# SegoleneMartin/transductive-CLIP

Measured on AMD Instinct MI355X. Metric: transductive tasks/sec (75-query EM-Dirichlet), higher is better.
Workload: dtype f32

## Files before the change

include/tclip.h:

```cpp
#ifndef TCLIP_H
#define TCLIP_H

#include <stddef.h>
#include <stdint.h>

#ifdef __cplusplus
extern "C" {
#endif

#define TCLIP_ABI_VERSION 5

enum {
    TCLIP_OK = 0,
    TCLIP_ERR_ARG = 1,
    TCLIP_ERR_WORKSPACE = 2,
    TCLIP_ERR_HIP = 3,
    TCLIP_ERR_INDEX = 4
};

typedef struct tclip_problem {
    int32_t n_batches;
    int32_t tasks_per_batch;
    int32_t n_query;
    int32_t n_class;
// ... 81 lines not shown
    float alpha_value;
    float loss_weights[3];
    int32_t entropies[3];
} tclip_tim_params;
size_t tclip_alpha_tim_workspace_bytes(const tclip_problem* p);
int tclip_alpha_tim_run(const tclip_problem* p, const tclip_tim_params* prm, const float* x_q, const float* x_s,
                        const int64_t* y_s, float* weights, float* logits_q, int32_t* preds, float* criterions,
                        void* workspace, size_t workspace_bytes, void* stream);

size_t tclip_laplacian_shot_workspace_bytes(const tclip_problem* p);
int tclip_laplacian_shot_run(const tclip_problem* p, const float* x_q, const float* x_s, const int64_t* y_s, int32_t knn,
                             double lmd, int32_t norm_type, float* unary, int32_t* neighbours, int32_t* preds_iter,
                             double* energies, void* workspace, size_t workspace_bytes, void* stream);

int tclip_argmax_rows(const float* x, int64_t n_rows, int32_t n_class, int32_t* labels, void* stream);

int tclip_probability_features(const float* visual, const float* text, int64_t n_rows, int32_t dim, int32_t n_class,
                               float temperature, float* out, void* stream);

#define TCLIP_VISUAL_SOFT_KMEANS 0
#define TCLIP_VISUAL_HARD_KMEANS 1
#define TCLIP_VISUAL_EM_GAUSSIAN 2
size_t tclip_visual_workspace_bytes(const tclip_problem* p, int32_t dim);
int tclip_kmeans_visual_run(const tclip_problem* p, int32_t dim, int32_t method, const float* x_q, const float* u0,
                            float temperature, float* u, float* v, float* w, int32_t* preds, float* criterions, void* workspace,
                            size_t workspace_bytes, void* stream);

int tclip_cluster_prototypes_visual(int32_t n_task, int32_t n_query, int32_t n_class, int32_t dim, const float* x_q,
                                    const int32_t* preds, int32_t* n_clusters, int32_t* cluster_ids, float* prototypes, void* stream);

int tclip_visual_init(const float* visual, const float* text, int64_t n_rows, int32_t dim, int32_t n_class,
                      float temperature, float* out, void* stream);

size_t tclip_paddle_visual_workspace_bytes(const tclip_problem* p, int32_t dim);
int tclip_paddle_visual_run(const tclip_problem* p, int32_t dim, const float* x_q, const float* x_s, const int64_t* y_s,
                            float lambd, float* u, float* v, float* w, int32_t* preds, void* workspace, size_t workspace_bytes,
                            void* stream);
size_t tclip_bdcspn_visual_workspace_bytes(const tclip_problem* p, int32_t dim);
int tclip_bdcspn_visual_run(const tclip_problem* p, int32_t dim, const float* x_q, const float* x_s, const int64_t* y_s, float temp,
                            int32_t norm_type, float* prototypes, float* u, int32_t* preds, void* workspace,
                            size_t workspace_bytes, void* stream);

int tclip_profile_enable(int on);
int tclip_profile_collect(double* mm_busy_ms, double* mm_launch_ms_sum, int64_t* mm_launches,
                          int64_t* element_updates);
int tclip_profile_last_kernels(double* busy_ms, double* launch_ms_sum, int64_t* launches, int64_t* element_updates);
int tclip_profile_last_split_sorts(int64_t* wave_iterations, int64_t* sorts);
int tclip_debug_set_split_keep_placement(int32_t on);

int tclip_debug_set_probe_chunks(int32_t chunks);

int tclip_debug_set_dead_head(int32_t iterations);

int tclip_debug_set_rowset_min_rows(int32_t rows);

int tclip_debug_set_mm_split(int32_t mode);

int tclip_debug_set_fixed_k_kernels(int32_t on);

int tclip_debug_set_kmeans_tile(int32_t mode);

int tclip_selftest_primitives(uint64_t* mismatches);

#ifdef __cplusplus
}
#endif
#endif
```

transductive-clip_amd/csrc/tclip_kernels.hip:

```cpp
#include <hip/hip_runtime.h>
#include <stdint.h>
#include <stdio.h>
#include <stdlib.h>
#include <string.h>

#include <algorithm>
#include <mutex>
#include <utility>
#include <vector>

#include "../../include/tclip.h"
#include "tclip_device.h"
#include "tclip_pk.h"
#include "tclip_selftest_inputs.h"

namespace tclip {

constexpr int kG64MinK = 897;

__global__ void k_log_features(const float* __restrict__ x, float* __restrict__ out, size_t n, int32_t* __restrict__ nonfinite) {
    bool bad = false;
    for (size_t i = (size_t)blockIdx.x * blockDim.x + threadIdx.x; i < n; i += (size_t)gridDim.x * blockDim.x) {
        const float v = log_f32(x[i] + kEpsF);
        out[i] = v;
// ... 278 lines not shown
        if (kCov) {
            y[row * K + d] = c / (s < kEpsF ? kEpsF : s);
        } else if (paddle == 2) {
            y[row * K + d] = s / c;
        } else if (sup && paddle) {
            y[row * K + d] = (s + sup[row * K + d]) / (c + cnt[row]);
        } else if (sup) {
            const float w = 1.0f / (cnt[row] + c);
            y[row * K + d] = w * (sup[row * K + d] + s);
        } else {
            y[row * K + d] = s / (c < kEpsF ? kEpsF : c);
        }
    }
}

__device__ __forceinline__ int lanes_below_mask(unsigned long long m, int lane) { return __popcll(m & ((1ull << lane) - 1ull)); }

__global__ void k_build_rows(const uint8_t* __restrict__ live, const int32_t* __restrict__ cache_len, int n_rows,
                             int n_checks, int32_t* __restrict__ dead_rows, int32_t* __restrict__ live_rows,
                             int32_t* __restrict__ n_dead, int32_t* __restrict__ n_live) {
    const int i = blockIdx.x * blockDim.x + threadIdx.x;
    const bool in = i < n_rows;
    const bool alive = in && live[i];
    const bool need = in && !alive && n_checks > 0 && cache_len[i] < n_checks;
    const unsigned long long ml = __ballot(alive), md = __ballot(need);
    const int lane64 = threadIdx.x & 63;
    int base_l = 0, base_d = 0;
    if (lane64 == 0) {
        if (ml) base_l = atomicAdd(n_live, __popcll(ml));
        if (md) base_d = atomicAdd(n_dead, __popcll(md));
    }
    base_l = __shfl(base_l, 0, 64);
    base_d = __shfl(base_d, 0, 64);
    if (alive) live_rows[base_l + lanes_below_mask(ml, lane64)] = i;
    if (need) dead_rows[base_d + lanes_below_mask(md, lane64)] = i;
}

struct MMArgs {
    float* alpha;
    float* beta_dead;
    const float* y;
    const uint8_t* live;
    int32_t* cache_len;
    double* cache;
    double* rowpart;
    const int32_t* rows;
    const int32_t* n_rows;
    const int32_t* stop;
    unsigned long long* work_counter;
    int32_t* next_rows;
    int32_t* next_count;
    int K, rows_per_batch, chunk, l0, l1, has_check, n_checks;
    int keep_placement;
};

constexpr int kYRegsMaxE = 16;
template <int E, int G>
__device__ __forceinline__ int elem_of(int e, int lane) {
    if constexpr (G == 64) return (lane >> 5) * (E * 32) + e * 32 + (lane & 31);
    else return e * G + lane;
}
template <int E, int G>
__host__ __device__ constexpr int full_registers(int K) {
    if constexpr (G == 64) return K > E * 32 ? (K - E * 32) / 32 : 0;
    else return K / G;
}

template <int E, int G = kGroup, int kRegsMaxE = kYRegsMaxE>
struct RowY {
    static constexpr bool kInRegs = E <= kRegsMaxE;
    float r[kInRegs ? E : 1];
    const float* g;
    int lane, K, n_full;
    __device__ __forceinline__ void load(const float* row_y, int lane_, int K_) {
        g = row_y; lane = lane_; K = K_; n_full = full_registers<E, G>(K_);
        if (kInRegs) {
#pragma unroll
            for (int e = 0; e < (kInRegs ? E : 1); e++) {
                const int d = elem_of<E, G>(e, lane);
                r[e] = d < K ? (g ? g[d] : -10.0f) : 0.0f;
            }
        }
    }
    __device__ __forceinline__ void fetch_all(float (&out)[E]) const {
        if (!g) {
#pragma unroll
            for (int e = 0; e < E; e++) out[e] = -10.0f;
            return;
        }
        if constexpr (G == 64) {
            const float* base = g;
            asm volatile("" : "+s"(base));
            const __amdgpu_buffer_rsrc_t rsrc = __builtin_amdgcn_make_buffer_rsrc((void*)base, 0, K * 4, 0x00020000);
            int voff = elem_of<E, G>(0, lane) * 4;
            asm volatile("" : "+v"(voff));
#pragma unroll
            for (int e = 0; e < E; e++) out[e] = __builtin_bit_cast(float, __builtin_amdgcn_raw_buffer_load_b32(rsrc, voff + e * 128, 0, 0));
        } else {
#pragma unroll
            for (int e = 0; e < E; e++) out[e] = get(e);
        }
    }
    __device__ __forceinline__ float get(int e) const {
        if (kInRegs) return r[kInRegs ? e : 0];
        if (!g) return -10.0f;
        const int d = elem_of<E, G>(e, lane);
// ... 158 lines not shown
    if constexpr (G == kGroup) return group_sum_torch<E, false, sure_registers<E, G, KC>()>(x, K, lane);
    else if constexpr (G == 64) return group_sum_torch_64<E, false, sure_registers<E, G, KC>()>(x, K, lane);
    else return group_sum_torch_g<E, G, false, sure_registers<E, G, KC>()>(x, K, lane);
}

template <int E, int G>
__device__ __forceinline__ void mm_iterate(float (&beta)[E], const RowY<E, G>& yv, int K, int lane,
                                           const LogTabEntry* tab, float* queue, bool measure, double& num,
                                           double& den) {
    const float s = row_sum_torch_all<E, G>(beta, K, lane);
    bool in_domain = fast_range_f32(s) && s <= 0x1p40f;
    uint32_t largest = 0u;
#pragma unroll
    for (int e = 0; e < E; e++) largest = max(largest, f32_bits(beta[e]));
    in_domain = in_domain & mm_fast_domain_of_max_bits(largest);
    if (__builtin_expect(!__all(in_domain), 0)) {
        const float psi_s = digamma_f32(s);
#pragma unroll
        for (int e = 0; e < E; e++) {
            const float nb = mm_update_generic(beta[e], yv.get(e), psi_s);
            const bool ok = elem_of<E, G>(e, lane) < K;
            if (measure && ok) {
                const double df = (double)nb - (double)beta[e];
                num += df * df;
                den += (double)beta[e] * (double)beta[e];
            }
            beta[e] = ok ? nb : 0.0f;
        }
        return;
    }
    const float psi_s = digamma_pos_f32(s, tab);
    int n_big = 0;
#pragma unroll
    for (int e = 0; e < E; e++) {
        const float x1 = beta[e] + 1.0f;
        const bool big = x1 >= 2.3f;
        const unsigned long long m = __ballot(big);
        if (big) queue[n_big + lanes_below(m)] = x1;
        n_big += __popcll(m);
    }
    __builtin_amdgcn_wave_barrier();
    const unsigned long long active = __ballot(true);
    const int rank = lanes_below(active), n_active = __popcll(active);
    for (int start = 0; start < n_big; start += n_active) {
        const int idx = start + rank;
        const float v = idx < n_big ? queue[idx] : 8.0f;
        const float r = lgamma_big_dense(v);
        if (idx < n_big) queue[idx] = r;
    }
    __builtin_amdgcn_wave_barrier();
    if (n_big == 0) mm_apply_updates_small<E, G>(beta, yv, K, lane, psi_s, tab, measure, num, den);
    else mm_apply_updates<E, G>(beta, yv, K, lane, psi_s, tab, queue, 0, measure, num, den);
    __builtin_amdgcn_wave_barrier();
}

constexpr int kProbeChunks = 2;
constexpr int kMaxCycle = 64;

constexpr int kMMWavesLarge = 3;
constexpr int kMMWavesSmall = 4;
template <int E, int G>
__global__ __launch_bounds__(256, (E > 16 ? kMMWavesLarge : kMMWavesSmall)) void k_mm_probe(MMArgs a) {
    __shared__ LogTabEntry tab[16];
    __shared__ double cyc[256 / G][kMaxCycle][2];
    __shared__ float lg_queue[4][64 * E];
    load_log_table(tab);
    float* queue = lg_queue[threadIdx.x >> 6];
    const int lane = threadIdx.x & (G - 1);
    const int group = threadIdx.x / G;
    const int groups_per_block = blockDim.x / G;
    const int n = *a.n_rows;
    const int K = a.K;
    for (int i = blockIdx.x * groups_per_block + group; i < n; i += gridDim.x * groups_per_block) {
        const int row = a.rows[i];
        if (a.stop[row / a.rows_per_batch]) continue;
        const int have = a.cache_len[row];
        if (have != a.chunk + 1) {
            if (a.next_rows && have < a.n_checks && lane == 0) a.next_rows[atomicAdd(a.next_count, 1)] = row;
            continue;
        }
        const float* ref = a.beta_dead + (size_t)row * K;
        float beta[E];
        RowY<E, G> yv;
        yv.load(nullptr, lane, K);
#pragma unroll
        for (int e = 0; e < E; e++) {
            const int d = elem_of<E, G>(e, lane);
            beta[e] = d < K ? ref[d] : 0.0f;
        }
        int period = 0;
        for (int j = 0; j < kMaxCycle && period == 0; j++) {
            double pn = 0.0, pd = 0.0;
            mm_iterate<E, G>(beta, yv, K, lane, tab, queue, true, pn, pd);
            pn = group_sum_f64_g<G>(pn);
            pd = group_sum_f64_g<G>(pd);
            if (lane == 0) { cyc[group][j][0] = pn; cyc[group][j][1] = pd; }
            bool same = true;
#pragma unroll
            for (int e = 0; e < E; e++) {
                const int d = elem_of<E, G>(e, lane);
                if (d < K) same = same && (beta[e] == ref[d]);
            }
            const unsigned long long bal = __ballot(same);
            constexpr unsigned long long kAll = G == 64 ? ~0ull : (1ull << (G & 63)) - 1ull;
            const unsigned long long mine = (bal >> ((threadIdx.x & 63) & ~(G - 1))) & kAll;
            if (mine == kAll) period = j + 1;
        }
        if (period && lane == 0) {
            for (int m = a.chunk + 1; m < a.n_checks; m++) {
                const int j = (50 * (m + 1) - (a.l1 + 1)) % period;
                double* c = a.cache + ((size_t)row * a.n_checks + m) * 2;
                c[0] = cyc[group][j][0];
                c[1] = cyc[group][j][1];
            }
            a.cache_len[row] = a.n_checks;
        }
        if (!period && a.next_rows && lane == 0) a.next_rows[atomicAdd(a.next_count, 1)] = row;
    }
}

constexpr int kDeadHead = 12;
static_assert(kDeadHead <= 18, "the last snapshot (32 iterations after the head) must lie at or before the first checkpoint (iteration 50)");
template <int E, int G>
__global__ __launch_bounds__(256, (E > 16 ? kMMWavesLarge : kMMWavesSmall)) void k_mm_probe_head(MMArgs a) {
    __shared__ LogTabEntry tab[16];
    __shared__ double cyc[256 / G][kMaxCycle][2];
    __shared__ float lg_queue[4][64 * E];
    load_log_table(tab);
    float* queue = lg_queue[threadIdx.x >> 6];
    const int lane = threadIdx.x & (G - 1);
    const int group = threadIdx.x / G;
    const int groups_per_block = blockDim.x / G;
    const int n = *a.n_rows;
    const int K = a.K;
    for (int i = blockIdx.x * groups_per_block + group; i < n; i += gridDim.x * groups_per_block) {
        const int row = a.rows[i];
        if (a.stop[row / a.rows_per_batch]) continue;
        if (a.cache_len[row] != 0) {
            if (lane == 0) a.next_rows[atomicAdd(a.next_count, 1)] = row;
            continue;
        }
        float* ref = a.beta_dead + (size_t)row * K;
        float* ref8 = const_cast<float*>(a.y) + (size_t)row * K;
        float beta[E];
        RowY<E, G> yv;
        yv.load(nullptr, lane, K);
#pragma unroll
        for (int e = 0; e < E; e++) {
            const int d = elem_of<E, G>(e, lane);
            beta[e] = d < K ? ref[d] : 0.0f;
        }
        int period = 0, js = 0, base = 0;
        bool have8 = false;
        constexpr unsigned long long kAll = G == 64 ? ~0ull : (1ull << (G & 63)) - 1ull;
        const int shift = (threadIdx.x & 63) & ~(G - 1);
        for (int j = 0; j < kMaxCycle && period == 0; j++) {
            double pn = 0.0, pd = 0.0;
            mm_iterate<E, G>(beta, yv, K, lane, tab, queue, true, pn, pd);
            pn = group_sum_f64_g<G>(pn);
            pd = group_sum_f64_g<G>(pd);
            if (lane == 0) { cyc[group][j][0] = pn; cyc[group][j][1] = pd; }
            bool same = true, same8 = have8;
#pragma unroll
            for (int e = 0; e < E; e++) {
                const int d = elem_of<E, G>(e, lane);
                if (d < K) same = same && (beta[e] == ref[d]);
            }
            if (have8) {
#pragma unroll
                for (int e = 0; e < E; e++) {
                    const int d = elem_of<E, G>(e, lane);
                    if (d < K) same8 = same8 && (beta[e] == ref8[d]);
                }
            }
            const bool hit = ((__ballot(same) >> shift) & kAll) == kAll, hit8 = ((__ballot(same8) >> shift) & kAll) == kAll;
            if (hit) {
                period = j + 1 - js;
                base = js;
            } else if (have8 && hit8) {
                period = j + 1 - 8;
                base = 8;
            } else if (j + 1 == 8 || j + 1 == 32) {
                float* dst = j + 1 == 8 ? ref8 : ref;
#pragma unroll
                for (int e = 0; e < E; e++) {
                    const int d = elem_of<E, G>(e, lane);
                    if (d < K) dst[d] = beta[e];
                }
                if (j + 1 == 8) have8 = true;
                else js = 32;
            }
        }
        if (period && lane == 0) {
            for (int m = 0; m < a.n_checks; m++) {
                const int t = 50 * (m + 1) - a.l0;
                const int j = base + (t - base) % period;
                double* c = a.cache + ((size_t)row * a.n_checks + m) * 2;
                c[0] = cyc[group][j][0];
                c[1] = cyc[group][j][1];
            }
            a.cache_len[row] = a.n_checks;
        }
        if (!period && lane == 0) a.next_rows[atomicAdd(a.next_count, 1)] = row;
    }
}

struct QueueCtl { int count[2][8]; int bad; float rowsum[2][64]; float psi[2][64]; };

template <int E, int G, int KC = 0>
__device__ __forceinline__ float row_sum_torch(const float (&x)[E], int K, int lane) {
    if constexpr (G == kGroup) return group_sum_torch<E, true, sure_registers<E, G, KC>()>(x, K, lane);
    else if constexpr (G == 64) return group_sum_torch_64<E, true, sure_registers<E, G, KC>()>(x, K, lane);
    else return group_sum_torch_g<E, G, true, sure_registers<E, G, KC>()>(x, K, lane);
}

template <int E, int W, int R, int G, int KC = 0>
__device__ __forceinline__ void mm_iterate_block(float (&beta)[R][E], const RowY<E, G> (&yv)[R], int K, int lane,
                                                 const bool (&active)[R], const LogTabEntry* tab, float* queue, QueueCtl* ctl,
                                                 int turn, bool measure, double (&num)[R], double (&den)[R]) {
    constexpr int kGroups = (64 / G) * W;
    const int wave = threadIdx.x >> 6, lane64 = threadIdx.x & 63;
    float s[R];
    bool in_domain = true;
    float* slice = queue + wave * (64 * E * R);
    int base[R + 1];
    base[0] = 0;
#pragma unroll
    for (int r = 0; r < R; r++) {
        s[r] = 16.0f;
        if (active[r]) {
            s[r] = row_sum_torch<E, G, KC>(beta[r], K, lane);
            in_domain = in_domain && (lane != 0 || (fast_range_f32(s[r]) && s[r] <= 0x1p40f));
            uint32_t largest = 0u;
#pragma unroll
            for (int e = 0; e < E; e++) largest = max(largest, f32_bits(beta[r][e]));
            in_domain = in_domain & mm_fast_domain_of_max_bits(largest);
        }
        if (lane == 0) ctl->rowsum[turn & 1][r * kGroups + (threadIdx.x / G)] = s[r];
        int idx = base[r];
#pragma unroll
        for (int e = 0; e < E; e++) {
            const float x1 = beta[r][e] + 1.0f;
            const bool big = active[r] && x1 >= 2.3f;
// ... 1510 lines not shown
        }
        if (x1 >= 2.3f) b2 += f32_bits(digamma_rec_acc_ge23(x1)) != f32_bits(acc);
        b2 += f32_bits(psip.x) != f32_bits(digamma_pos_f32(xp.x, tab)) || f32_bits(psip.y) != f32_bits(digamma_pos_f32(xp.y, tab));
    }
    for (uint32_t m = tid; m < (1u << 24); m += nth) {
        const float x = bits_f32(0x3f800000u + m);
        const f2 r = pk_sqrt_torch_inrange(f2{x, x * 0x1p-60f});
        b4 += f32_bits(r.x) != f32_bits(sqrt_torch_inrange_f32(x)) || f32_bits(r.y) != f32_bits(sqrt_torch_inrange_f32(x * 0x1p-60f));
        b4 += f32_bits(sqrt_torch_inrange_dev(x * 0x1p61f)) != f32_bits(sqrt_torch_inrange_f32(x * 0x1p61f));
    }
    for (int e = -100 + (int)tid; e <= 100; e += (int)nth) {
        const float x = bits_f32((uint32_t)(127 + e) << 23);
        b4 += f32_bits(sqrt_torch_inrange_dev(x)) != f32_bits(sqrt_torch_inrange_f32(x));
        b4 += f32_bits(pk_sqrt_torch_inrange(pk(x)).y) != f32_bits(sqrt_torch_inrange_f32(x));
    }
    atomicAdd(&out[0], b0); atomicAdd(&out[1], b1); atomicAdd(&out[2], b2);
    atomicAdd(&out[3], b3); atomicAdd(&out[4], b4); atomicAdd(&out[5], b5);
    for (int f = 0; f < kSelfTestFunctions; f++) {
        unsigned long long c = 0;
        for (uint32_t i = tid; i < kSelfTestCount; i += nth) c += selftest_term(f, i, tab);
        atomicAdd(&out[6 + f], c);
    }
}

thread_local char g_err[512] = "";

static int fail(int code, const char* fmt, const char* detail = "") {
    snprintf(g_err, sizeof g_err, fmt, detail);
    return code;
}

#define TCLIP_HIP(call)                                                                     \
    do {                                                                                    \
        hipError_t e_ = (call);                                                             \
        if (e_ != hipSuccess) return fail(TCLIP_ERR_HIP, #call ": %s", hipGetErrorString(e_)); \
    } while (0)

static size_t align_up(size_t x) { return (x + 255) & ~(size_t)255; }

struct Profile {
    bool on = false;
    std::vector<hipEvent_t> ev;
    std::vector<uint8_t> kind;
    size_t used = 0;
    unsigned long long* counter = nullptr;
    double last_busy[2] = {0, 0}, last_sum[2] = {0, 0};
    int64_t last_launches[2] = {0, 0}, last_updates[2] = {0, 0};
    int64_t last_split_iterations = 0, last_split_sorts = 0;
};
static thread_local bool g_last_mm_was_split = false;
thread_local Profile g_prof;
static int g_probe_chunks = kProbeChunks;
static int g_dead_head = kDeadHead;
static int g_rowset_min_rows = -1;
static int g_mm_split = -1;
static int g_split_keep_placement = 1;

static hipEvent_t prof_event() {
    if (g_prof.used == g_prof.ev.size()) {
        hipEvent_t e;
        if (hipEventCreate(&e) != hipSuccess) return nullptr;
        g_prof.ev.push_back(e);
    }
    return g_prof.ev[g_prof.used++];
}

constexpr int kDecideSlices = 64;
struct Layout {
    size_t logz, y, alpha_old, beta_dead, sup, cnt, cs, live, rowc, logit0, cache, cache_len, rowpart, mm_rows,
        mm_rows2, mm_rows3, dead_counts, cls, n_live, live_rows, counts, flags, stop, ratio, dpart, total;
    int n_checks;
};

static int n_chunks_of(int iter_mm) { return iter_mm <= 51 ? 1 : 1 + (iter_mm - 51 + 49) / 50; }
static int n_checks_of(int iter_mm) { return iter_mm <= 50 ? 0 : (iter_mm - 1) / 50; }

static Layout make_layout(const tclip_problem& p) {
    Layout L;
    const size_t T = (size_t)p.n_batches * p.tasks_per_batch, K = p.n_class, Q = p.n_query;
    const bool zs = p.n_support == 0;
    L.n_checks = n_checks_of(p.iter_mm);
    size_t o = 0;
    auto take = [&](size_t bytes) { size_t r = o; o += align_up(bytes); return r; };
    L.logz = take(T * Q * K * 4);
    L.y = take(T * K * K * 4);
    L.alpha_old = take(T * K * K * 4);
    L.beta_dead = take(zs ? T * K * K * 4 : 0);
    L.sup = take(zs ? 0 : T * K * K * 4);
    L.cnt = take(zs ? 0 : T * K * 4);
    L.cs = take(T * K * 4);
    L.live = take(T * K);
    L.rowc = take(T * K * 4);
    L.logit0 = take(T * Q * K * 4);
    L.cache = take(zs ? T * K * (size_t)L.n_checks * 16 : 0);
    L.cache_len = take(T * K * 4);
    L.rowpart = take(T * K * 16);
    L.mm_rows = take(T * K * 4);
    L.mm_rows2 = take(zs ? T * K * 4 : 0);
    L.mm_rows3 = take(zs ? T * K * 4 : 0);
    L.dead_counts = take(((size_t)n_chunks_of(p.iter_mm) + 3) * 4);
    L.cls = take(zs ? T * K * 2 : 0);
    L.n_live = take(zs ? T * 4 : 0);
    L.live_rows = take(T * K * 4);
    L.counts = take(256);
    L.flags = take(256);
    L.stop = take((size_t)p.n_batches * 4);
// ... 572 lines not shown
    int32_t* counts = (int32_t*)(ws + L.counts);
    int32_t* flags = (int32_t*)(ws + L.flags);
    int32_t* stop = (int32_t*)(ws + L.stop);
    float* ratio = (float*)(ws + L.ratio);
    double* dpart = (double*)(ws + L.dpart);
    const int n_chunks = n_chunks_of(p.iter_mm);
    const int n_checks = zs ? L.n_checks : 0;

    TCLIP_HIP(hipMemsetAsync(flags, 0, 256, st));
    if (q_src.idx) {
        const size_t rows = (size_t)T * Q;
        hipLaunchKernelGGL(k_gather_log_features, dim3((unsigned)(rows > 65536 ? 65536 : rows)), dim3(256), 0, st, q_src, Q, K, rows, u, logz, flags);
    } else {
        hipLaunchKernelGGL(k_log_features, dim3(ew_grid(TQK)), dim3(256), 0, st, q_src.base, logz, TQK, flags);
        hipLaunchKernelGGL(k_copy, dim3(ew_grid(TQK)), dim3(256), 0, st, q_src.base, u, TQK);
    }
    hipLaunchKernelGGL(k_fill, dim3(ew_grid(TKK)), dim3(256), 0, st, alpha, 1.0f, TKK);
    hipLaunchKernelGGL(k_fill, dim3(ew_grid(TKK)), dim3(256), 0, st, alpha_old, 1.0f, TKK);
    hipLaunchKernelGGL(k_fill, dim3(ew_grid(TK)), dim3(256), 0, st, v, 0.0f, (size_t)TK);
    TCLIP_HIP(hipMemsetAsync(cache_len, 0, (size_t)TK * 4, st));
    if (!zs) {
        hipLaunchKernelGGL(k_support_stats, dim3(K, T), dim3(128), (size_t)S * sizeof(int), st, s_src, y_s, S, K, 1, sup, cnt);
    }
    {
        TCLIP_HIP(hipMemsetAsync(counts, 0, 256, st));
        hipLaunchKernelGGL(k_one_row_list, dim3(1), dim3(1), 0, st, mm_rows, counts + 2);
        dispatch_E<LaunchRowConsts>(K, 1, st, (const float*)alpha, (const int32_t*)mm_rows, (const int32_t*)(counts + 2), K, rowc);
        hipLaunchKernelGGL(k_broadcast_first, dim3(ew_grid((size_t)TK)), dim3(256), 0, st, rowc, (size_t)TK);
        TCLIP_HIP(hipMemsetAsync(live, 1, (size_t)TK, st));
        hipLaunchKernelGGL(k_build_rows, dim3((TK + 255) / 256), dim3(256), 0, st, live, cache_len, TK, 0, mm_rows,
                           live_rows, counts, counts + 1);
        hipLaunchKernelGGL(k_init_logits, dim3(ew_grid(TQK)), dim3(256), 0, st, (const float*)rowc, (const int32_t*)flags, Q, K, TQK, logit0);
        dispatch_E<LaunchLogits>(K, TK > 262144 ? 262144 : TK, st, (const float*)alpha, (const float*)logz, (const float*)rowc,
                                 (const int32_t*)live_rows, (const int32_t*)(counts + 1), Q, K, logit0, (const int32_t*)flags);
    }

    for (int it = 0; it < p.iters; it++) {
        hipLaunchKernelGGL(k_cluster_sizes, dim3((TK + 255) / 256), dim3(256), 0, st, (const float*)u, T, Q, K, zs ? 1 : 0,
                           cs, live, v, cache_len);
        launch_mstats(st, (const float*)u, (const float*)logz, (const float*)cs, (const uint8_t*)live, (const float*)sup, (const float*)cnt, T, Q, K, y, 0,
                      !zs || it == 0, (zs && it > 0) ? (int16_t*)(ws + L.cls) : nullptr, (zs && it > 0) ? (int32_t*)(ws + L.n_live) : nullptr);
        TCLIP_HIP(hipMemsetAsync(counts, 0, 256, st));
        TCLIP_HIP(hipMemsetAsync(dead_counts, 0, ((size_t)n_chunks + 3) * 4, st));
        TCLIP_HIP(hipMemsetAsync(stop, 0, (size_t)B * 4, st));
        hipLaunchKernelGGL(k_build_rows, dim3((TK + 255) / 256), dim3(256), 0, st, (const uint8_t*)live,
                           (const int32_t*)cache_len, TK, n_checks, dead_list[0], live_rows, dead_counts, counts + 1);
        for (int c = 0; c < n_chunks; c++) {
            MMArgs a;
            a.alpha = alpha; a.beta_dead = beta_dead; a.y = y; a.live = live; a.cache_len = cache_len;
            a.cache = cache; a.rowpart = rowpart; a.rows = mm_rows; a.n_rows = counts; a.stop = stop;
            a.next_rows = nullptr; a.next_count = nullptr;
            a.K = K; a.rows_per_batch = N * K; a.chunk = c;
            a.keep_placement = g_split_keep_placement;
            a.l0 = c == 0 ? 0 : 50 * c + 1;
            a.l1 = 50 * (c + 1) < p.iter_mm - 1 ? 50 * (c + 1) : p.iter_mm - 1;
            a.has_check = (a.l1 > 0 && a.l1 % 50 == 0) ? 1 : 0;
            a.n_checks = n_checks > 0 ? n_checks : 1;
            const bool split = g_mm_split < 0 ? it >= kSplitFrom : (g_mm_split >= 100 ? it >= g_mm_split - 100 : g_mm_split != 0);
            const bool split_runs = split && mm_has_split(K);
            a.work_counter = g_prof.on ? g_prof.counter + (split_runs ? 1 : 0) : nullptr;
            hipEvent_t e0 = g_prof.on ? prof_event() : nullptr, e1 = g_prof.on ? prof_event() : nullptr;
            if (e0 && e1) TCLIP_HIP(hipEventRecord(e0, st));
            a.rows = live_rows; a.n_rows = counts + 1;
            g_last_mm_was_split = false;
            launch_mm(split ? kMMSplit : kMMLive, K, TK, st, a);
            if (e0 && e1) {
                TCLIP_HIP(hipEventRecord(e1, st));
                if (g_prof.kind.size() < g_prof.used / 2) g_prof.kind.resize(g_prof.used / 2);
                g_prof.kind[g_prof.used / 2 - 1] = g_last_mm_was_split ? 1 : 0;
            }
            if (split_runs != g_last_mm_was_split) return fail(TCLIP_ERR_ARG, "internal: mm_has_split disagrees with launch_mm");
            if (zs && a.has_check) {
                a.rows = dead_list[c & 1]; a.n_rows = dead_counts + c; a.work_counter = nullptr;
                if (c == 0 && g_dead_head > 0 && g_probe_chunks > 0) {
                    MMArgs h = a;
                    h.l0 = 0; h.l1 = g_dead_head - 1; h.has_check = 0; h.next_rows = nullptr; h.next_count = nullptr;
                    launch_mm(kMMDead, K, TK, st, h);
                    h.l0 = g_dead_head; h.next_rows = head_back; h.next_count = dead_counts + n_chunks + 2;
                    launch_mm(kMMProbeHead, K, TK, st, h);
                    a.rows = head_back; a.n_rows = dead_counts + n_chunks + 2;
                }
                const bool more = c + 1 < a.n_checks, probe = c < g_probe_chunks && more;
                int32_t* next_rows = more ? dead_list[(c + 1) & 1] : nullptr;
                int32_t* next_count = more ? dead_counts + c + 1 : nullptr;
                a.next_rows = probe ? nullptr : next_rows; a.next_count = probe ? nullptr : next_count;
                launch_mm(kMMDead, K, TK, st, a);
                a.next_rows = next_rows; a.next_count = next_count;
                if (probe) launch_mm(kMMProbe, K, TK, st, a);
            }
            const bool two_stage = a.has_check && N * K > 16384;
            if (two_stage)
                hipLaunchKernelGGL(k_mm_decide_partial, dim3(kDecideSlices, B), dim3(256), 0, st, (const double*)rowpart,
                                   (const double*)cache, (const uint8_t*)live, N * K, a.n_checks, c, (const int32_t*)stop, dpart);
            hipLaunchKernelGGL(k_mm_decide, dim3(B), dim3(1024), 0, st, (const double*)rowpart, (const double*)cache,
                               (const uint8_t*)live, N * K, a.n_checks, c, a.has_check, a.l1, c == n_chunks - 1 ? 1 : 0,
                               p.iter_mm, stop, mm_iters + it, p.iters, (const double*)(two_stage ? dpart : nullptr),
                               kDecideSlices);
        }
        {
            const int g8 = (TK + 7) / 8 > 65535 * 8 ? 65535 * 8 : (TK + 7) / 8;
            dispatch_E<LaunchRowConsts>(K, g8 > 4096 ? 4096 : g8, st, (const float*)alpha, (const int32_t*)live_rows,
                                        (const int32_t*)(counts + 1), K, rowc);
            dispatch_E<LaunchLogits>(K, TK > kLogitsGrid ? kLogitsGrid : TK, st, (const float*)alpha, (const float*)logz, (const float*)rowc,
                                     (const int32_t*)live_rows, (const int32_t*)(counts + 1), Q, K, logit0, (const int32_t*)nullptr);
        }
        hipLaunchKernelGGL(k_softmax, dim3((T * Q * 16 + 255) / 256), dim3(256), 0, st, (const float*)logit0, (const float*)v,
// ... 534 lines not shown
}

int tclip_argmax_rows(const float* x, int64_t n_rows, int32_t n_class, int32_t* labels, void* stream) {
    if (!x || !labels || n_rows < 0 || n_class < 1) return fail(TCLIP_ERR_ARG, "bad argument to tclip_argmax_rows");
    if (n_rows == 0) return TCLIP_OK;
    hipLaunchKernelGGL(k_argmax_rows, dim3((unsigned)((n_rows + 255) / 256)), dim3(256), 0, (hipStream_t)stream, x, (long)n_rows,
                       n_class, labels);
    TCLIP_HIP(hipGetLastError());
    return TCLIP_OK;
}

int tclip_probability_features(const float* visual, const float* text, int64_t n_rows, int32_t dim, int32_t n_class,
                               float temperature, float* out, void* stream) {
    if (!visual || !text || !out || n_rows < 0 || dim < 1 || n_class < 1) return fail(TCLIP_ERR_ARG, "bad argument to tclip_probability_features");
    if (n_rows == 0) return TCLIP_OK;
    const size_t lds = ((size_t)dim + (size_t)n_class) * sizeof(float);
    if (lds > 60000 || n_rows > 0x7fffffff) return fail(TCLIP_ERR_ARG, "dim + n_class must be <= 15000");
    hipLaunchKernelGGL(k_probability_features<false>, dim3((unsigned)n_rows), dim3(256), lds, (hipStream_t)stream, visual, text,
                       dim, n_class, temperature, out);
    TCLIP_HIP(hipGetLastError());
    return TCLIP_OK;
}

int tclip_debug_set_rowset_min_rows(int32_t rows) {
    g_rowset_min_rows = rows;
    return TCLIP_OK;
}

int tclip_debug_set_kmeans_tile(int32_t mode) {
    g_kmeans_tile = mode;
    return TCLIP_OK;
}

int tclip_debug_set_fixed_k_kernels(int32_t on) {
    g_fixed_k_kernels = on;
    return TCLIP_OK;
}

int tclip_debug_set_mm_split(int32_t mode) {
    g_mm_split = mode;
    return TCLIP_OK;
}

int tclip_debug_set_split_keep_placement(int32_t on) {
    g_split_keep_placement = on != 0;
    return TCLIP_OK;
}

int tclip_debug_set_dead_head(int32_t iterations) {
    if (iterations > 18) return fail(TCLIP_ERR_ARG, "tclip_debug_set_dead_head: at most 18 iterations");
    g_dead_head = iterations < 0 ? kDeadHead : iterations;
    return TCLIP_OK;
}
int tclip_debug_set_probe_chunks(int32_t chunks) {
    g_probe_chunks = chunks < 0 ? kProbeChunks : chunks;
    return TCLIP_OK;
}

int tclip_profile_enable(int on) {
    if (on && !g_prof.counter) {
        TCLIP_HIP(hipMalloc((void**)&g_prof.counter, 4 * sizeof(unsigned long long)));
        TCLIP_HIP(hipMemset(g_prof.counter, 0, 4 * sizeof(unsigned long long)));
    }
    g_prof.on = on != 0;
    return TCLIP_OK;
}

static double union_ms(std::vector<std::pair<float, float>>& iv) {
    std::sort(iv.begin(), iv.end());
    double busy = 0.0, cur_lo = 0.0, cur_hi = -1.0;
    for (auto& x : iv) {
        if (cur_hi < cur_lo || x.first > cur_hi) {
            if (cur_hi >= cur_lo) busy += cur_hi - cur_lo;
            cur_lo = x.first;
            cur_hi = x.second;
        } else if (x.second > cur_hi) {
            cur_hi = x.second;
        }
    }
    if (cur_hi >= cur_lo) busy += cur_hi - cur_lo;
    return busy;
}
int tclip_profile_collect(double* mm_busy_ms, double* mm_launch_ms_sum, int64_t* mm_launches,
                          int64_t* element_updates) {
    TCLIP_HIP(hipDeviceSynchronize());
    std::vector<std::pair<float, float>> iv, ivk[2];
    double sum = 0.0;
    for (int k = 0; k < 2; k++) { g_prof.last_sum[k] = 0.0; g_prof.last_launches[k] = 0; }
    for (size_t i = 0; i + 1 < g_prof.used; i += 2) {
        float t0 = 0.f, t1 = 0.f;
        TCLIP_HIP(hipEventElapsedTime(&t0, g_prof.ev[0], g_prof.ev[i]));
        TCLIP_HIP(hipEventElapsedTime(&t1, g_prof.ev[0], g_prof.ev[i + 1]));
        iv.emplace_back(t0, t1);
        sum += (double)t1 - (double)t0;
        const int k = i / 2 < g_prof.kind.size() ? g_prof.kind[i / 2] : 0;
        ivk[k].emplace_back(t0, t1);
        g_prof.last_sum[k] += (double)t1 - (double)t0;
        g_prof.last_launches[k]++;
    }
    const double busy = union_ms(iv);
    for (int k = 0; k < 2; k++) g_prof.last_busy[k] = union_ms(ivk[k]);
    if (mm_busy_ms) *mm_busy_ms = busy;
    if (mm_launch_ms_sum) *mm_launch_ms_sum = sum;
    if (mm_launches) *mm_launches = (int64_t)(g_prof.used / 2);
    unsigned long long c[4] = {0, 0, 0, 0};
    if (g_prof.counter) {
// ... 114 lines not shown
```

transductive-clip_amd/tclip_amd/_capi.py:

```python
import ctypes
import os

_HERE = os.path.dirname(os.path.abspath(__file__))
LIB_PATH = os.path.join(_HERE, "libtclip.so")


class Problem(ctypes.Structure):
    _fields_ = [(n, ctypes.c_int32) for n in (
        "n_batches", "tasks_per_batch", "n_query", "n_class", "n_support", "iters", "iter_mm", "lambd", "hard")]


class TaskSource(ctypes.Structure):
    _fields_ = [(n, ctypes.c_void_p) for n in ("table_q", "q_idx", "table_s", "s_idx", "cols")]


class TimParams(ctypes.Structure):
    _fields_ = [("lr", ctypes.c_double), ("temp", ctypes.c_float), ("alpha_value", ctypes.c_float),
                ("loss_weights", ctypes.c_float * 3), ("entropies", ctypes.c_int32 * 3)]


_P = ctypes.c_void_p
_SIGNATURES = {
    "tclip_abi_version": (ctypes.c_int, []),
    "tclip_last_error": (ctypes.c_char_p, []),
    "tclip_workspace_bytes": (ctypes.c_size_t, [ctypes.POINTER(Problem)]),
    "tclip_em_dirichlet_run": (ctypes.c_int, [ctypes.POINTER(Problem)] + [_P] * 10 + [ctypes.c_size_t, _P]),
    "tclip_em_dirichlet_run_tasks": (ctypes.c_int, [ctypes.POINTER(Problem), ctypes.POINTER(TaskSource)] + [_P] * 8 + [ctypes.c_size_t, _P]),
    "tclip_prototype_workspace_bytes": (ctypes.c_size_t, [ctypes.c_int32] * 3),
    "tclip_cluster_prototypes": (ctypes.c_int, [ctypes.c_int32] * 3 + [_P] * 6 + [ctypes.c_size_t, _P]),
    "tclip_match_clusters_host": (ctypes.c_int, [ctypes.c_int32] * 3 + [_P] * 5 + [ctypes.c_int32, _P, _P]),
    "tclip_match_clusters_host_strided": (ctypes.c_int, [ctypes.c_int32] * 3 + [_P] * 5 + [ctypes.c_int32, ctypes.c_int32, _P, _P]),
    "tclip_host_threads": (ctypes.c_int, []),
    "tclip_gather_rows": (ctypes.c_int, [_P, ctypes.c_int64, ctypes.c_int32, _P, ctypes.c_int64, _P, _P]),
    "tclip_soft_kmeans_workspace_bytes": (ctypes.c_size_t, [ctypes.POINTER(Problem)]),
    "tclip_soft_kmeans_run": (ctypes.c_int, [ctypes.POINTER(Problem), _P, ctypes.c_float, _P, _P, _P, _P, ctypes.c_size_t, _P]),
    "tclip_em_gaussian_run": (ctypes.c_int, [ctypes.POINTER(Problem), _P, ctypes.c_float, _P, _P, _P, _P, _P, ctypes.c_size_t, _P]),
    "tclip_em_gaussian_cov_run": (ctypes.c_int, [ctypes.POINTER(Problem), _P, _P, _P, _P, _P, _P, _P, ctypes.c_size_t, _P]),
    "tclip_paddle_workspace_bytes": (ctypes.c_size_t, [ctypes.POINTER(Problem)]),
    "tclip_paddle_run": (ctypes.c_int, [ctypes.POINTER(Problem), _P, _P, _P, ctypes.c_float, _P, _P, _P, _P, _P, ctypes.c_size_t, _P]),
    "tclip_alpha_tim_workspace_bytes": (ctypes.c_size_t, [ctypes.POINTER(Problem)]),
    "tclip_alpha_tim_run": (ctypes.c_int, [ctypes.POINTER(Problem), ctypes.POINTER(TimParams)] + [_P] * 8 + [ctypes.c_size_t, _P]),
    "tclip_laplacian_shot_workspace_bytes": (ctypes.c_size_t, [ctypes.POINTER(Problem)]),
    "tclip_laplacian_shot_run": (ctypes.c_int, [ctypes.POINTER(Problem), _P, _P, _P, ctypes.c_int32, ctypes.c_double, ctypes.c_int32,
                                                _P, _P, _P, _P, _P, ctypes.c_size_t, _P]),
    "tclip_bdcspn_workspace_bytes": (ctypes.c_size_t, [ctypes.POINTER(Problem)]),
    "tclip_bdcspn_run": (ctypes.c_int, [ctypes.POINTER(Problem), _P, _P, _P, ctypes.c_float, ctypes.c_int32, _P, _P, _P, _P, ctypes.c_size_t, _P]),
    "tclip_hard_kmeans_workspace_bytes": (ctypes.c_size_t, [ctypes.POINTER(Problem)]),
    "tclip_hard_kmeans_run": (ctypes.c_int, [ctypes.POINTER(Problem), _P, _P, _P, _P, _P, _P, ctypes.c_size_t, _P]),
    "tclip_kl_kmeans_run": (ctypes.c_int, [ctypes.POINTER(Problem), _P, _P, _P, _P, _P, _P, ctypes.c_size_t, _P]),
    "tclip_argmax_rows": (ctypes.c_int, [_P, ctypes.c_int64, ctypes.c_int32, _P, _P]),
    "tclip_probability_features": (ctypes.c_int, [_P, _P, ctypes.c_int64, ctypes.c_int32, ctypes.c_int32, ctypes.c_float, _P, _P]),
    "tclip_visual_workspace_bytes": (ctypes.c_size_t, [ctypes.POINTER(Problem), ctypes.c_int32]),
    "tclip_kmeans_visual_run": (ctypes.c_int, [ctypes.POINTER(Problem), ctypes.c_int32, ctypes.c_int32, _P, _P, ctypes.c_float,
                                               _P, _P, _P, _P, _P, _P, ctypes.c_size_t, _P]),
    "tclip_cluster_prototypes_visual": (ctypes.c_int, [ctypes.c_int32] * 4 + [_P] * 6),
    "tclip_visual_init": (ctypes.c_int, [_P, _P, ctypes.c_int64, ctypes.c_int32, ctypes.c_int32, ctypes.c_float, _P, _P]),
    "tclip_paddle_visual_workspace_bytes": (ctypes.c_size_t, [ctypes.POINTER(Problem), ctypes.c_int32]),
    "tclip_paddle_visual_run": (ctypes.c_int, [ctypes.POINTER(Problem), ctypes.c_int32, _P, _P, _P, ctypes.c_float, _P, _P, _P, _P,
                                               _P, ctypes.c_size_t, _P]),
    "tclip_bdcspn_visual_workspace_bytes": (ctypes.c_size_t, [ctypes.POINTER(Problem), ctypes.c_int32]),
    "tclip_bdcspn_visual_run": (ctypes.c_int, [ctypes.POINTER(Problem), ctypes.c_int32, _P, _P, _P, ctypes.c_float, ctypes.c_int32,
                                               _P, _P, _P, _P, ctypes.c_size_t, _P]),
    "tclip_selftest_primitives": (ctypes.c_int, [ctypes.POINTER(ctypes.c_uint64)]),
    "tclip_profile_enable": (ctypes.c_int, [ctypes.c_int]),
    "tclip_debug_set_probe_chunks": (ctypes.c_int, [ctypes.c_int32]),
    "tclip_debug_set_dead_head": (ctypes.c_int, [ctypes.c_int32]),
    "tclip_debug_set_rowset_min_rows": (ctypes.c_int, [ctypes.c_int32]),
    "tclip_debug_set_mm_split": (ctypes.c_int, [ctypes.c_int32]),
    "tclip_debug_set_split_keep_placement": (ctypes.c_int, [ctypes.c_int32]),
    "tclip_debug_set_fixed_k_kernels": (ctypes.c_int, [ctypes.c_int32]),
    "tclip_debug_set_kmeans_tile": (ctypes.c_int, [ctypes.c_int32]),
    "tclip_profile_last_kernels": (ctypes.c_int, [ctypes.POINTER(ctypes.c_double), ctypes.POINTER(ctypes.c_double),
                                                  ctypes.POINTER(ctypes.c_int64), ctypes.POINTER(ctypes.c_int64)]),
    "tclip_check_task_indices": (ctypes.c_int, [_P, ctypes.c_int64, ctypes.c_int64, _P, ctypes.c_int64, ctypes.c_int32, _P]),
    "tclip_profile_last_split_sorts": (ctypes.c_int, [ctypes.POINTER(ctypes.c_int64), ctypes.POINTER(ctypes.c_int64)]),
    "tclip_profile_collect": (ctypes.c_int, [ctypes.POINTER(ctypes.c_double), ctypes.POINTER(ctypes.c_double),
                                             ctypes.POINTER(ctypes.c_int64), ctypes.POINTER(ctypes.c_int64)]),
}
EXPORTS = tuple(_SIGNATURES)
_lib = None


def lib():
    global _lib
    if _lib is None:
        path = os.environ.get("TCLIP_LIB") or LIB_PATH
        if not os.path.exists(path):
            raise RuntimeError(
                f"{path} is missing: build it with `python transductive-clip_amd/build.py` "
                "(there is no CPU or PyTorch fallback for the EM-Dirichlet path)")
        import torch
        hip_rt = os.path.join(os.path.dirname(torch.__file__), "lib", "libamdhip64.so")
        if os.path.exists(hip_rt):
            ctypes.CDLL(hip_rt, mode=ctypes.RTLD_GLOBAL)
        l = ctypes.CDLL(path)
        for name, (res, args) in _SIGNATURES.items():
            fn = getattr(l, name)
            fn.restype, fn.argtypes = res, args
        if l.tclip_abi_version() != 5:
            raise RuntimeError("libtclip.so ABI version mismatch")
        _lib = l
    return _lib


def _strip_comments(text):
    out, i, n = [], 0, len(text)
    while i < n:
        c = text[i]
        if c == '"' or c == "'":
            j = i + 1
            while j < n and text[j] != c:
                j += 2 if text[j] == "\\" else 1
            out.append(text[i:j + 1])
            i = j + 1
        elif text.startswith("//", i):
            j = text.find("\n", i)
            i = n if j < 0 else j
        elif text.startswith("/*", i):
            j = text.find("*/", i + 2)
# ... 23 lines not shown
```

transductive-clip_amd/tclip_amd/engine.py:

```python
import ctypes

import torch

from . import _capi


def _ptr(t):
    return ctypes.c_void_p(t.data_ptr()) if t is not None else None


def _stream():
    return ctypes.c_void_p(torch.cuda.current_stream().cuda_stream)


def _require_cuda(t, name):
    if not t.is_cuda:
        raise RuntimeError(f"{name} must live on the GPU: the EM-Dirichlet engine has no CPU path")


class EMDirichletResult:
    __slots__ = ("u", "v", "alpha", "preds", "criterions", "mm_iters")

    def __init__(self, **kw):
        for k, val in kw.items():
# ... 377 lines not shown
    new_preds = torch.empty(T, Q, dtype=torch.int32)
    acc = torch.empty(T, dtype=torch.float32)
    rc = lib.tclip_match_clusters_host_strided(T, Q, K, _ptr(preds_h), _ptr(nc_h), _ptr(ids_h), _ptr(rows_h), _ptr(y_h),
                                               int(bool(graph_matching)), used, _ptr(new_preds), _ptr(acc))
    _capi.check(rc, "tclip_match_clusters_host_strided")
    return acc, new_preds


def clustering_accuracy_visual(x_q, preds, y_q, text, T, graph_matching=True):
    _require_cuda(x_q, "x_q")
    x_q = x_q.contiguous().float()
    n_task, Q, D = x_q.shape
    dev = x_q.device
    text = text.to(dev).contiguous().float()
    if text.dim() != 2 or text.shape[1] != D:
        raise ValueError(f"text features must be (K, {D}) for {D}-dim embeddings, got {tuple(text.shape)}")
    K = text.shape[0]
    lib = _capi.lib()
    cmax = min(Q, K)
    with torch.cuda.device(dev):
        preds = preds.to(dev).int().contiguous()
        n_clusters = torch.empty(n_task, dtype=torch.int32, device=dev)
        ids = torch.empty(n_task, cmax, dtype=torch.int32, device=dev)
        protos = torch.ones(n_task, cmax, D, device=dev)
        rc = lib.tclip_cluster_prototypes_visual(n_task, Q, K, D, _ptr(x_q), _ptr(preds), _ptr(n_clusters), _ptr(ids), _ptr(protos),
                                                 _stream())
        _capi.check(rc, "tclip_cluster_prototypes_visual")
        probs = torch.empty(n_task, cmax, K, device=dev)
        rc = lib.tclip_probability_features(_ptr(protos), _ptr(text), ctypes.c_int64(n_task * cmax), ctypes.c_int32(D),
                                            ctypes.c_int32(K), ctypes.c_float(float(T)), _ptr(probs), _stream())
        _capi.check(rc, "tclip_probability_features")
    return _match(lib, n_task, Q, K, preds, n_clusters, ids, probs, y_q, graph_matching, cmax, dev)


def gather_rows(table, idx):
    _require_cuda(table, "table")
    table = table.contiguous().float()
    idx = _index_tensor(idx.reshape(-1), table.shape[0], table.device, "idx")
    out = torch.empty(idx.numel(), table.shape[1], device=table.device)
    with torch.cuda.device(table.device):
        rc = _capi.lib().tclip_gather_rows(_ptr(table), table.shape[0], table.shape[1], _ptr(idx), idx.numel(), _ptr(out), _stream())
    _capi.check(rc, "tclip_gather_rows")
    return out


def debug_set_probe_chunks(chunks=-1):
    _capi.check(_capi.lib().tclip_debug_set_probe_chunks(int(chunks)), "tclip_debug_set_probe_chunks")


def debug_set_dead_head(iterations=-1):
    _capi.check(_capi.lib().tclip_debug_set_dead_head(int(iterations)), "tclip_debug_set_dead_head")


def debug_set_rowset_min_rows(rows=-1):
    _capi.check(_capi.lib().tclip_debug_set_rowset_min_rows(int(rows)), "tclip_debug_set_rowset_min_rows")


def profile_enable(on=True):
    _capi.check(_capi.lib().tclip_profile_enable(int(bool(on))), "tclip_profile_enable")


def profile_collect():
    busy, total, n, upd = ctypes.c_double(0), ctypes.c_double(0), ctypes.c_int64(0), ctypes.c_int64(0)
    _capi.check(_capi.lib().tclip_profile_collect(ctypes.byref(busy), ctypes.byref(total), ctypes.byref(n),
                                                  ctypes.byref(upd)), "tclip_profile_collect")
    return busy.value, total.value, n.value, upd.value


def profile_last_kernels():
    busy, total = (ctypes.c_double * 2)(), (ctypes.c_double * 2)()
    n, upd = (ctypes.c_int64 * 2)(), (ctypes.c_int64 * 2)()
    _capi.check(_capi.lib().tclip_profile_last_kernels(busy, total, n, upd), "tclip_profile_last_kernels")
    return {name: (busy[i], total[i], n[i], upd[i]) for i, name in enumerate(("k_mm_live", "k_mm_split"))}


def profile_last_split_sorts():
    it, so = ctypes.c_int64(0), ctypes.c_int64(0)
    _capi.check(_capi.lib().tclip_profile_last_split_sorts(ctypes.byref(it), ctypes.byref(so)), "tclip_profile_last_split_sorts")
    return it.value, so.value
```

Measured before the change: 160.6.

## Collapse dead-row MM probe iterations onto a few distinct beta values

In the cycle-detection probe for stalled (dead) rows, each row's beta entries are checked to see whether they take at most eight distinct values. If they do, the minorize-maximize update is computed once per distinct value and scattered back with ds_bpermute, and the period check compares a single value instead of every element. This targets repeated per-element digamma/lgamma work and the full-row comparisons on rows that have collapsed to a few values. In exchange it adds detection ballot loops, extra register state and fallback paths when the domain checks fail. It is enabled by default through a new debug knob.

```diff
diff --git a/include/tclip.h b/include/tclip.h
--- a/include/tclip.h
+++ b/include/tclip.h
@@ -157,6 +157,8 @@
 
 int tclip_debug_set_dead_head(int32_t iterations);
 
+int tclip_debug_set_dead_collapse(int32_t max_values);
+
 int tclip_debug_set_rowset_min_rows(int32_t rows);
 
 int tclip_debug_set_mm_split(int32_t mode);
diff --git a/transductive-clip_amd/csrc/tclip_kernels.hip b/transductive-clip_amd/csrc/tclip_kernels.hip
--- a/transductive-clip_amd/csrc/tclip_kernels.hip
+++ b/transductive-clip_amd/csrc/tclip_kernels.hip
@@ -354,6 +354,7 @@
     int32_t* next_count;
     int K, rows_per_batch, chunk, l0, l1, has_check, n_checks;
     int keep_placement;
+    int collapse_max;
 };
 
 constexpr int kYRegsMaxE = 16;
@@ -618,6 +619,98 @@
     if (n_big == 0) mm_apply_updates_small<E, G>(beta, yv, K, lane, psi_s, tab, measure, num, den);
     else mm_apply_updates<E, G>(beta, yv, K, lane, psi_s, tab, queue, 0, measure, num, den);
     __builtin_amdgcn_wave_barrier();
+}
+
+constexpr int kCollapseMax = 8;
+template <int E>
+struct CollapsedRow {
+    float val;
+    uint32_t at[(E + 3) / 4];
+    int epoch;
+    bool on;
+};
+
+template <int E, int G>
+__device__ __forceinline__ bool collapse_detect(const float (&beta)[E], int K, int lane, int max_values, CollapsedRow<E>& c) {
+    static_assert(E <= 32 && kCollapseMax <= 16, "one pending bit per register; the list fits the smallest lane group");
+    constexpr unsigned long long kAll = G == 64 ? ~0ull : (1ull << (G & 63)) - 1ull;
+    const int shift = (threadIdx.x & 63) & ~(G - 1);
+    uint32_t pend = 0u;
+#pragma unroll
+    for (int e = 0; e < E; e++) pend |= elem_of<E, G>(e, lane) < K ? 1u << e : 0u;
+#pragma unroll
+    for (int q = 0; q < (E + 3) / 4; q++) c.at[q] = 0u;
+    uint32_t mine = 0u, first = 0u;
+    int n = 0;
+    c.val = 0.0f;
+    for (;;) {
+        const unsigned long long m = (__ballot(pend != 0u) >> shift) & kAll;
+        if (m == 0ull) break;
+        if (n == max_values) return false;
+        uint32_t cand = 0u;
+#pragma unroll
+        for (int e = E - 1; e >= 0; e--) cand = ((pend >> e) & 1u) ? f32_bits(beta[e]) : cand;
+        const uint32_t v = (uint32_t)__shfl((int)cand, shift + __ffsll(m) - 1, 64);
+        const uint32_t addr = (uint32_t)(shift + n) * 4u;
+#pragma unroll
+        for (int e = 0; e < E; e++) {
+            const bool hit = f32_bits(beta[e]) == v;
+            c.at[e / 4] |= hit ? addr << (8 * (e % 4)) : 0u;
+            pend &= hit ? ~(1u << e) : ~0u;
+        }
+        if (n == 0) first = v;
+        if (lane == n) mine = v;
+        n++;
+    }
+    c.val = bits_f32(lane < n ? mine : first);
+    return true;
+}
+
+template <int E, int G>
+__device__ __forceinline__ bool mm_iterate_collapsed(float (&beta)[E], int K, int lane, const LogTabEntry* tab, CollapsedRow<E>& c,
+                                                     bool measure, double& num, double& den) {
+    const float s = row_sum_torch_all<E, G>(beta, K, lane);
+    const bool in_domain = fast_range_f32(s) && s <= 0x1p40f && mm_fast_domain_of_max_bits(f32_bits(c.val));
+    if (__builtin_expect(!__all(in_domain), 0)) return false;
+    const float psi_s = digamma_pos_f32(s, tab);
+    const float a = c.val, x1 = a + 1.0f;
+    const bool big = x1 >= 2.3f;
+    float nv;
+    if (__ballot(big) == 0ull) {
+        nv = pk_mm_update_stage2(pk_mm_update_stage1_small(f2{a, a}, pk(-10.0f), pk(psi_s), tab)).x;
+    } else {
+        const float lg = lgamma_big_dense(big ? x1 : 8.0f);
+        nv = pk_mm_update_stage2(pk_mm_update_stage1(f2{a, a}, pk(-10.0f), pk(psi_s), pk(big ? lg : 0.0f), tab)).x;
+    }
+    const int n_full = full_registers<E, G>(K);
+#pragma unroll
+    for (int e = 0; e < E; e++) {
+        const int addr = (int)((c.at[e / 4] >> (8 * (e % 4))) & 0xffu);
+        const float nb = bits_f32((uint32_t)__builtin_amdgcn_ds_bpermute(addr, (int)f32_bits(nv)));
+        const bool ok = e < n_full || elem_of<E, G>(e, lane) < K;
+        if (measure && ok) {
+            const double df = (double)nb - (double)beta[e];
+            num += df * df;
+            den += (double)beta[e] * (double)beta[e];
+        }
+        beta[e] = ok ? nb : 0.0f;
+    }
+    c.val = nv;
+    return true;
+}
+
+template <int E, int G>
+__device__ __forceinline__ void probe_iterate(float (&beta)[E], const RowY<E, G>& yv, int K, int lane, const LogTabEntry* tab,
+                                              float* queue, int collapse_max, CollapsedRow<E>& c, double& num, double& den) {
+    if (collapse_max > 0) {
+        if (!c.on) {
+            c.on = collapse_detect<E, G>(beta, K, lane, collapse_max, c);
+            c.epoch++;
+        }
+        if (__all(c.on) && mm_iterate_collapsed<E, G>(beta, K, lane, tab, c, true, num, den)) return;
+        c.on = false;
+    }
+    mm_iterate<E, G>(beta, yv, K, lane, tab, queue, true, num, den);
 }
 
 constexpr int kProbeChunks = 2;
@@ -654,18 +747,27 @@
             const int d = elem_of<E, G>(e, lane);
             beta[e] = d < K ? ref[d] : 0.0f;
         }
+        CollapsedRow<E> col;
+        col.on = a.collapse_max > 0 && collapse_detect<E, G>(beta, K, lane, a.collapse_max, col);
+        col.epoch = 0;
+        const uint32_t ref_val = f32_bits(col.val);
+        const bool ref_listed = col.on;
         int period = 0;
         for (int j = 0; j < kMaxCycle && period == 0; j++) {
             double pn = 0.0, pd = 0.0;
-            mm_iterate<E, G>(beta, yv, K, lane, tab, queue, true, pn, pd);
+            probe_iterate<E, G>(beta, yv, K, lane, tab, queue, a.collapse_max, col, pn, pd);
             pn = group_sum_f64_g<G>(pn);
             pd = group_sum_f64_g<G>(pd);
             if (lane == 0) { cyc[group][j][0] = pn; cyc[group][j][1] = pd; }
             bool same = true;
-#pragma unroll
-            for (int e = 0; e < E; e++) {
-                const int d = elem_of<E, G>(e, lane);
-                if (d < K) same = same && (beta[e] == ref[d]);
+            if (ref_listed && col.on && col.epoch == 0) {
+                same = f32_bits(col.val) == ref_val;
+            } else {
+#pragma unroll
+                for (int e = 0; e < E; e++) {
+                    const int d = elem_of<E, G>(e, lane);
+                    if (d < K) same = same && (beta[e] == ref[d]);
+                }
             }
             const unsigned long long bal = __ballot(same);
             constexpr unsigned long long kAll = G == 64 ? ~0ull : (1ull << (G & 63)) - 1ull;
@@ -720,23 +822,36 @@
         bool have8 = false;
         constexpr unsigned long long kAll = G == 64 ? ~0ull : (1ull << (G & 63)) - 1ull;
         const int shift = (threadIdx.x & 63) & ~(G - 1);
+        CollapsedRow<E> col;
+        col.on = a.collapse_max > 0 && collapse_detect<E, G>(beta, K, lane, a.collapse_max, col);
+        col.epoch = 0;
+        uint32_t snap_val = f32_bits(col.val), snap8_val = 0u;
+        int snap_epoch = col.on ? 0 : -1, snap8_epoch = -1;
         for (int j = 0; j < kMaxCycle && period == 0; j++) {
             double pn = 0.0, pd = 0.0;
-            mm_iterate<E, G>(beta, yv, K, lane, tab, queue, true, pn, pd);
+            probe_iterate<E, G>(beta, yv, K, lane, tab, queue, a.collapse_max, col, pn, pd);
             pn = group_sum_f64_g<G>(pn);
             pd = group_sum_f64_g<G>(pd);
             if (lane == 0) { cyc[group][j][0] = pn; cyc[group][j][1] = pd; }
             bool same = true, same8 = have8;
-#pragma unroll
-            for (int e = 0; e < E; e++) {
-                const int d = elem_of<E, G>(e, lane);
-                if (d < K) same = same && (beta[e] == ref[d]);
-            }
-            if (have8) {
+            if (col.on && col.epoch == snap_epoch) {
+                same = f32_bits(col.val) == snap_val;
+            } else {
 #pragma unroll
                 for (int e = 0; e < E; e++) {
                     const int d = elem_of<E, G>(e, lane);
-                    if (d < K) same8 = same8 && (beta[e] == ref8[d]);
+                    if (d < K) same = same && (beta[e] == ref[d]);
+                }
+            }
+            if (have8) {
+                if (col.on && col.epoch == snap8_epoch) {
+                    same8 = f32_bits(col.val) == snap8_val;
+                } else {
+#pragma unroll
+                    for (int e = 0; e < E; e++) {
+                        const int d = elem_of<E, G>(e, lane);
+                        if (d < K) same8 = same8 && (beta[e] == ref8[d]);
+                    }
                 }
             }
             const bool hit = ((__ballot(same) >> shift) & kAll) == kAll, hit8 = ((__ballot(same8) >> shift) & kAll) == kAll;
@@ -753,8 +868,15 @@
                     const int d = elem_of<E, G>(e, lane);
                     if (d < K) dst[d] = beta[e];
                 }
-                if (j + 1 == 8) have8 = true;
-                else js = 32;
+                if (j + 1 == 8) {
+                    have8 = true;
+                    snap8_val = f32_bits(col.val);
+                    snap8_epoch = col.on ? col.epoch : -1;
+                } else {
+                    js = 32;
+                    snap_val = f32_bits(col.val);
+                    snap_epoch = col.on ? col.epoch : -1;
+                }
             }
         }
         if (period && lane == 0) {
@@ -2371,6 +2493,7 @@
 thread_local Profile g_prof;
 static int g_probe_chunks = kProbeChunks;
 static int g_dead_head = kDeadHead;
+static int g_dead_collapse = kCollapseMax;
 static int g_rowset_min_rows = -1;
 static int g_mm_split = -1;
 static int g_split_keep_placement = 1;
@@ -3049,6 +3172,7 @@
             a.next_rows = nullptr; a.next_count = nullptr;
             a.K = K; a.rows_per_batch = N * K; a.chunk = c;
             a.keep_placement = g_split_keep_placement;
+            a.collapse_max = g_dead_collapse;
             a.l0 = c == 0 ? 0 : 50 * c + 1;
             a.l1 = 50 * (c + 1) < p.iter_mm - 1 ? 50 * (c + 1) : p.iter_mm - 1;
             a.has_check = (a.l1 > 0 && a.l1 % 50 == 0) ? 1 : 0;
@@ -3689,6 +3813,11 @@
     g_dead_head = iterations < 0 ? kDeadHead : iterations;
     return TCLIP_OK;
 }
+int tclip_debug_set_dead_collapse(int32_t max_values) {
+    if (max_values > kCollapseMax) return fail(TCLIP_ERR_ARG, "tclip_debug_set_dead_collapse: at most 8 values");
+    g_dead_collapse = max_values < 0 ? kCollapseMax : max_values;
+    return TCLIP_OK;
+}
 int tclip_debug_set_probe_chunks(int32_t chunks) {
     g_probe_chunks = chunks < 0 ? kProbeChunks : chunks;
     return TCLIP_OK;
diff --git a/transductive-clip_amd/tclip_amd/_capi.py b/transductive-clip_amd/tclip_amd/_capi.py
--- a/transductive-clip_amd/tclip_amd/_capi.py
+++ b/transductive-clip_amd/tclip_amd/_capi.py
@@ -65,6 +65,7 @@
     "tclip_profile_enable": (ctypes.c_int, [ctypes.c_int]),
     "tclip_debug_set_probe_chunks": (ctypes.c_int, [ctypes.c_int32]),
     "tclip_debug_set_dead_head": (ctypes.c_int, [ctypes.c_int32]),
+    "tclip_debug_set_dead_collapse": (ctypes.c_int, [ctypes.c_int32]),
     "tclip_debug_set_rowset_min_rows": (ctypes.c_int, [ctypes.c_int32]),
     "tclip_debug_set_mm_split": (ctypes.c_int, [ctypes.c_int32]),
     "tclip_debug_set_split_keep_placement": (ctypes.c_int, [ctypes.c_int32]),
diff --git a/transductive-clip_amd/tclip_amd/engine.py b/transductive-clip_amd/tclip_amd/engine.py
--- a/transductive-clip_amd/tclip_amd/engine.py
+++ b/transductive-clip_amd/tclip_amd/engine.py
@@ -453,6 +453,10 @@
     _capi.check(_capi.lib().tclip_debug_set_dead_head(int(iterations)), "tclip_debug_set_dead_head")
 
 
+def debug_set_dead_collapse(max_values=-1):
+    _capi.check(_capi.lib().tclip_debug_set_dead_collapse(int(max_values)), "tclip_debug_set_dead_collapse")
+
+
 def debug_set_rowset_min_rows(rows=-1):
     _capi.check(_capi.lib().tclip_debug_set_rowset_min_rows(int(rows)), "tclip_debug_set_rowset_min_rows")
 
```

Result: no change. 161.6, median of 6 (+0.7%).
